# 0xWOLAND/halo2-prover

Hardware: AMD Instinct MI355X
Metric: MSM+NTT field-ops/s (higher is better)
Workload: dtype u32 limbs (256-bit modular)

## Files before the change

halo2_prover_amd/csrc/h2_msm.hpp:

```cpp
#pragma once
#include "h2_curve29.hpp"
#include "h2_curve_quad.hpp"
#include "h2_tune.hpp"
#include <hip/hip_ext.h>
#include <algorithm>
#include <cstdlib>

namespace h2 {

#ifdef H2_TAIL_STAMPS
__device__ unsigned long long* h2_stamps;
#define H2_STAMP(slot)                                                                                              \
  do {                                                                                                              \
    if (threadIdx.x == 0) h2_stamps[((size_t)blockIdx.y * gridDim.x + blockIdx.x) * 16 + (slot)] = wall_clock64(); \
  } while (0)
#else
#define H2_STAMP(slot)
#endif

constexpr uint32_t MSM_SIGN = 0x80000000u;
constexpr uint32_t MSM_MAX_WINDOWS = 48;
constexpr uint32_t MSM_HOT_SPAN = 256;
constexpr uint32_t MSM_HOT_SEG = 128;
constexpr uint32_t MSM_NOT_HOT = 0xFFFFFFFFu;
constexpr uint32_t MSM_SORT_THREADS = 1024;
constexpr uint32_t MSM_CHUNK_WAVES = 3;
constexpr uint32_t MSM_MAX_C_ONE_LEVEL = 16;
constexpr uint32_t MSM_MAX_C = 19;

struct MsmGeom {
  uint32_t c;
  uint32_t W;
  uint32_t B;
  uint32_t nbits;
  uint32_t wbase, wextra;
  uint8_t off[MSM_MAX_WINDOWS];
  uint8_t width[MSM_MAX_WINDOWS];
};

inline MsmGeom msm_geometry(size_t n, uint32_t nbits) {
  uint32_t lg = 0;
  while (((size_t)1 << (lg + 1)) <= n) lg++;
  int c = (int)lg - (lg <= 15 ? 3 : 4);
  c = lg <= 20 ? std::min(c, 16) : 19;
  c = tune_int("H2_TUNE_C", c);
  if (c < 6) c = 6;
  if (c > (int)MSM_MAX_C) c = (int)MSM_MAX_C;
  MsmGeom g{};
  g.nbits = nbits;
  const uint32_t total = nbits + 1;
  g.W = (total + c - 1) / c;
  const uint32_t base = total / g.W, extra = total % g.W;
  g.wbase = base;
  g.wextra = extra;
  uint32_t o = 0;
  for (uint32_t w = 0; w < g.W; w++) {
    g.off[w] = (uint8_t)o;
    g.width[w] = (uint8_t)(base + (w < extra ? 1 : 0));
    o += g.width[w];
  }
  g.c = base + (extra ? 1 : 0);
  g.B = 1u << (g.c - 1);
  return g;
}

constexpr size_t MSM_TABLE_SCRATCH = 80;
template <class CV>
__global__ void __launch_bounds__(256)
msm_table_kernel(const U128* __restrict__ bases, U128* __restrict__ table, uint32_t* __restrict__ scratch, uint32_t n, MsmGeom g,
                 uint32_t* __restrict__ bad) {
  const uint32_t i = blockIdx.x * blockDim.x + threadIdx.x;
  if (i >= n) return;
  using B = typename CV::Base;
  using W = Fe29<B>;
  Affine<CV> p = affine_load<CV>(bases + 4 * (size_t)i);
  if (!p.is_identity()) {
    Fe<B> b;
#pragma unroll
    for (int k = 0; k < 8; k++) b.v[k] = CV::B(k);
    uint32_t rx[8], ry[8];
    fe_reduce_once<B>(rx, p.x.v, 0);
    fe_reduce_once<B>(ry, p.y.v, 0);
    bool ok = true;
#pragma unroll
    for (int k = 0; k < 8; k++) ok = ok && rx[k] == p.x.v[k] && ry[k] == p.y.v[k];
    if (!ok || fe_sqr(p.y) != fe_add(fe_mul(fe_sqr(p.x), p.x), b)) {
      atomicAdd(bad, 1u);
      p = Affine<CV>::identity();
    }
  }
  if (p.is_identity()) {
    for (uint32_t w = 0; w < g.W; w++) affine29_store_table<CV>(table + 4 * ((size_t)w * n + i), p);
    return;
  }
  auto slot_of = [&](uint32_t w) { return reinterpret_cast<uint32_t*>(table + 4 * ((size_t)w * n + i)); };
  auto scr_of = [&](uint32_t w) { return scratch + (MSM_TABLE_SCRATCH / 4) * ((size_t)w * n + i); };
  auto put9 = [](uint32_t* q, const W& v) {
#pragma unroll
    for (int l = 0; l < 9; l++) q[l] = (uint32_t)v.v[l];
  };
  auto get9 = [](const uint32_t* q) {
    W v;
#pragma unroll
    for (int l = 0; l < 9; l++) v.v[l] = (int32_t)q[l];
    return v;
  };
// ... 433 lines not shown
  return affine29_load<CV>(table + 4 * (size_t)(entry & ~MSM_SIGN), (entry & MSM_SIGN) != 0);
}

template <class CV>
__global__ void __launch_bounds__(256, MSM_CHUNK_WAVES)
msm_chunk_kernel(const U128* __restrict__ table, const U128* const* __restrict__ col_tables, uint32_t log_b,
                 const uint32_t* __restrict__ sorted_ref,
                 const uint32_t* __restrict__ chunk_first, const uint32_t* __restrict__ offsets, size_t K, uint32_t T_host,
                 uint32_t* __restrict__ bucket_sum, uint32_t* __restrict__ head, uint32_t* __restrict__ tail) {
  const uint32_t t = blockIdx.x * blockDim.x + threadIdx.x;
  const uint32_t E = offsets[K];
  const uint32_t T = msm_effective_t(E, T_host);
  const uint64_t lo64 = (uint64_t)t * T;
  if (lo64 >= E) return;
  const uint32_t lo = (uint32_t)lo64, hi = (uint32_t)min((uint64_t)E, lo64 + T);
  uint32_t key = chunk_first[t];
  uint32_t next = offsets[key + 1];
  if (col_tables) table = col_tables[key >> log_b];
  bool first = true;
  Xyzz29<CV> a = Xyzz29<CV>::identity();
  U128 quad = U128{0, 0, 0, 0};
  for (uint32_t e = lo; e < hi; e++) {
    if (e == lo || (e & 3u) == 0) quad = *reinterpret_cast<const U128*>(sorted_ref + (e & ~3u));
    const uint32_t sel = e & 3u;
    const uint32_t ref = sel == 0 ? quad.x : sel == 1 ? quad.y : sel == 2 ? quad.z : quad.w;
    if (e >= next) {
      if (first && offsets[key] != lo) xyzz29_store<CV>(head + XYZZ29_WORDS * (size_t)t, a);
      else xyzz29_store<CV>(bucket_sum + XYZZ29_WORDS * (size_t)key, a);
      first = false;
      a = Xyzz29<CV>::identity();
      do {
        key++;
        next = offsets[key + 1];
      } while (e >= next);
      if (col_tables) table = col_tables[key >> log_b];
    }
    a = xyzz29_add_affine(a, msm_fetch<CV>(table, ref));
  }
  const bool ends_here = next == hi;
  const bool starts_here = !first || offsets[key] == lo;
  if (starts_here && ends_here) xyzz29_store<CV>(bucket_sum + XYZZ29_WORDS * (size_t)key, a);
  else if (first) xyzz29_store<CV>(head + XYZZ29_WORDS * (size_t)t, a);
  else xyzz29_store<CV>(tail + XYZZ29_WORDS * (size_t)t, a);
}

template <class CV>
__device__ __forceinline__ Xyzz29<CV> xyzz_shfl_down(const Xyzz29<CV>& p, uint32_t delta) {
  Xyzz29<CV> r;
#pragma unroll
  for (int i = 0; i < 9; i++) {
    r.x.v[i] = __shfl_down(p.x.v[i], delta, 64);
    r.y.v[i] = __shfl_down(p.y.v[i], delta, 64);
    r.zz.v[i] = __shfl_down(p.zz.v[i], delta, 64);
    r.zzz.v[i] = __shfl_down(p.zzz.v[i], delta, 64);
  }
  return r;
}

__device__ __forceinline__ void h2_publish_release() {
  asm volatile("s_waitcnt vmcnt(0)" ::: "memory");
  __builtin_amdgcn_fence(__ATOMIC_RELEASE, "agent");
  asm volatile("s_waitcnt vmcnt(0)" ::: "memory");
}
__device__ __forceinline__ void h2_consume_acquire() {
  __builtin_amdgcn_fence(__ATOMIC_ACQUIRE, "agent");
  asm volatile("s_waitcnt vmcnt(0)" ::: "memory");
}

template <class CV>
__device__ __forceinline__ Xyzz29<CV> xyzz_fold_down(const Xyzz29<CV>& a, uint32_t d, uint32_t lane) {
  const Xyzz29<CV> o = xyzz_shfl_down(a, d);
  return lane < d ? xyzz29_add_quad(a, o) : a;
}

template <class CV>
__device__ __forceinline__ Xyzz29<CV> msm_piece(const uint32_t* __restrict__ head, const uint32_t* __restrict__ tail,
                                               uint32_t s, uint32_t j0, uint32_t T, uint32_t p) {
  const uint32_t j = j0 + p;
  const uint32_t* src = (p == 0 && s != j0 * T) ? tail : head;
  return xyzz29_load<CV>(src + XYZZ29_WORDS * (size_t)j);
}

template <class CV>
__global__ void __launch_bounds__(64)
msm_hot_reduce_kernel(const uint32_t* __restrict__ offsets, size_t K, uint32_t T_host, const uint32_t* __restrict__ hot_slot,
                      const uint32_t* __restrict__ tasks, const uint32_t* __restrict__ task_count, uint32_t max_tasks,
                      const uint32_t* __restrict__ head, const uint32_t* __restrict__ tail, uint32_t* __restrict__ hot_part) {
  __builtin_amdgcn_s_setprio(3);
  const uint32_t ntask = min(*task_count, max_tasks);
  const uint32_t T = msm_effective_t(offsets[K], T_host);
  const uint32_t quad = threadIdx.x >> 2;
  for (uint32_t t = blockIdx.x; t < ntask; t += gridDim.x) {
    const uint32_t key = tasks[2 * t], q = tasks[2 * t + 1];
    const uint32_t s = offsets[key], e = offsets[key + 1];
    const uint32_t j0 = s / T, span = (e - 1) / T - j0 + 1;
    const uint32_t lo = q * MSM_HOT_SEG, hi = min(span, lo + MSM_HOT_SEG);
    Xyzz29<CV> a = Xyzz29<CV>::identity();
    for (uint32_t p = lo + quad; p < hi; p += 16) a = xyzz29_add_quad(a, msm_piece<CV>(head, tail, s, j0, T, p));
    for (uint32_t d = 32; d >= 4; d >>= 1) a = xyzz_fold_down(a, d, threadIdx.x);
    if (threadIdx.x == 0) xyzz29_store<CV>(hot_part + XYZZ29_WORDS * (size_t)(hot_slot[key] + q), a);
  }
}

template <class CV>
__global__ void __launch_bounds__(256)
msm_fixup_kernel(const uint32_t* __restrict__ offsets, size_t K, uint32_t T_host, uint32_t log_g,
                 const uint32_t* __restrict__ bucket_sum, const uint32_t* __restrict__ head,
                 const uint32_t* __restrict__ tail, const uint32_t* __restrict__ hot_slot,
                 const uint32_t* __restrict__ hot_part, uint32_t* __restrict__ xsum) {
  __builtin_amdgcn_s_setprio(3);
  const uint32_t G = 1u << log_g;
  const uint32_t T = msm_effective_t(offsets[K], T_host);
  const size_t gt = (size_t)blockIdx.x * blockDim.x + threadIdx.x;
  const size_t key = gt >> log_g;
  const uint32_t lane = (uint32_t)gt & (G - 1);
  const uint32_t quad = lane >> 2, nquad = G >> 2;
  const bool live = key < K;
  Xyzz29<CV> x = Xyzz29<CV>::identity();
  if (live) {
    const uint32_t s = offsets[key], e = offsets[key + 1];
    if (e > s) {
      const uint32_t j0 = s / T, j1 = (e - 1) / T;
      if (j0 == j1) {
        if (quad == 0) x = xyzz29_load<CV>(bucket_sum + XYZZ29_WORDS * key);
      } else if (hot_slot[key] != MSM_NOT_HOT) {
        const uint32_t nseg = (j1 - j0 + 1 + MSM_HOT_SEG - 1) / MSM_HOT_SEG;
        const uint32_t* part = hot_part + XYZZ29_WORDS * (size_t)hot_slot[key];
        for (uint32_t q = quad; q < nseg; q += nquad) x = xyzz29_add_quad(x, xyzz29_load<CV>(part + XYZZ29_WORDS * (size_t)q));
      } else if (quad <= j1 - j0) {
        Xyzz29<CV> nxt = msm_piece<CV>(head, tail, s, j0, T, quad);
        for (uint32_t p = quad; p <= j1 - j0; p += nquad) {
          const Xyzz29<CV> cur = nxt;
          if (p + nquad <= j1 - j0) nxt = msm_piece<CV>(head, tail, s, j0, T, p + nquad);
          x = xyzz29_add_quad(x, cur);
        }
      }
    }
  }
  for (uint32_t d = G >> 1; d >= 4; d >>= 1) x = xyzz_fold_down(x, d, lane);
  if (live && lane == 0) xyzz29_store<CV>(xsum + XYZZ29_WORDS * key, x);
}

H2_HD bool msm_special_predoubled(uint32_t log_b, uint32_t lb) {
  const uint32_t hb = log_b - lb, ndig = ((hb + 1) >> 1) ? ((hb + 1) >> 1) : 1u;
  return lb >= 2 * ndig;
}
template <class CV>
__global__ void __launch_bounds__(256)
msm_rowcol_kernel(const uint32_t* __restrict__ xsum, uint32_t* __restrict__ rc, uint32_t* __restrict__ done,
                  uint32_t log_b, uint32_t lb, U128* zero_ptr = nullptr, uint32_t zero_u128 = 0) {
  __builtin_amdgcn_s_setprio(3);
  __shared__ uint32_t xw[3][XYZZ29_WORDS];
  const uint32_t col = blockIdx.y;
  if (blockIdx.x == 0 && threadIdx.x == 0) done[col] = 0;
  if (zero_ptr) {
    const uint32_t nthr = gridDim.x * gridDim.y * blockDim.x;
    for (uint32_t i = (blockIdx.y * gridDim.x + blockIdx.x) * blockDim.x + threadIdx.x; i < zero_u128; i += nthr)
      zero_ptr[i] = U128{0, 0, 0, 0};
  }
  const uint32_t rows = 1u << (log_b - lb), cols = 1u << lb;
  const bool is_row = blockIdx.x < rows;
  const uint32_t first = is_row ? blockIdx.x * cols : blockIdx.x - rows;
  const uint32_t stride = is_row ? 1u : cols, len = is_row ? cols : rows;
  const uint32_t* base = xsum + XYZZ29_WORDS * ((size_t)col << log_b);
  const uint32_t quad = threadIdx.x >> 2, nq = blockDim.x >> 2, lane = threadIdx.x & 63u, wave = threadIdx.x >> 6;
  Xyzz29<CV> a = quad < len ? xyzz29_load<CV>(base + XYZZ29_WORDS * (size_t)(first + quad * stride)) : Xyzz29<CV>::identity();
  if (quad + nq < len) {
    Xyzz29<CV> nxt = xyzz29_load<CV>(base + XYZZ29_WORDS * (size_t)(first + (quad + nq) * stride));
    for (uint32_t j = quad + nq; j < len; j += nq) {
      const Xyzz29<CV> cur = nxt;
      if (j + nq < len) nxt = xyzz29_load<CV>(base + XYZZ29_WORDS * (size_t)(first + (j + nq) * stride));
      a = xyzz29_add_quad(a, cur);
    }
  }
  for (uint32_t d = 32; d >= 4; d >>= 1) a = xyzz_fold_down(a, d, lane);
  if (blockDim.x > 64) {
    if (wave > 0 && lane == 0) xyzz29_store<CV>(xw[wave - 1], a);
    __syncthreads();
    if (wave > 0) return;
    const uint32_t nw = blockDim.x >> 6;
    if (quad >= 1) a = quad < nw ? xyzz29_load<CV>(xw[quad - 1]) : Xyzz29<CV>::identity();
    for (uint32_t d = 2 * nw; d >= 4; d >>= 1) a = xyzz_fold_down(a, d, lane);
  }
  if (is_row || (blockIdx.x == rows + cols - 1 && msm_special_predoubled(log_b, lb)))
    for (uint32_t k = 0; k < lb; k++) a = xyzz29_double_quad(a);
  if (threadIdx.x == 0) xyzz29_store<CV>(rc + XYZZ29_WORDS * ((size_t)col * (rows + cols) + blockIdx.x), a);
}
inline uint32_t msm_rowcol_waves(uint32_t log_b, uint32_t lb, size_t m) {
  const uint32_t rows = 1u << (log_b - lb), cols = 1u << lb;
  const uint32_t shortest = rows < cols ? rows : cols;
  uint32_t nw = 1;
  while (nw < 4 && shortest >= 64 * nw && (size_t)(rows + cols) * m * (2 * nw) <= 1024) nw *= 2;
  return nw;
}

template <class CV>
__device__ __forceinline__ Xyzz29<CV> xyzz29_pick(uint32_t dig, const Xyzz29<CV>& p1, const Xyzz29<CV>& p2, const Xyzz29<CV>& p3) {
  const int32_t m1 = -(int32_t)(dig == 1), m2 = -(int32_t)(dig == 2), m3 = -(int32_t)(dig == 3);
  Xyzz29<CV> r;
#pragma unroll
  for (int i = 0; i < 9; i++) {
    r.x.v[i] = (m1 & p1.x.v[i]) | (m2 & p2.x.v[i]) | (m3 & p3.x.v[i]);
    r.y.v[i] = (m1 & p1.y.v[i]) | (m2 & p2.y.v[i]) | (m3 & p3.y.v[i]);
    r.zz.v[i] = (m1 & p1.zz.v[i]) | (m2 & p2.zz.v[i]) | (m3 & p3.zz.v[i]);
    r.zzz.v[i] = (m1 & p1.zzz.v[i]) | (m2 & p2.zzz.v[i]) | (m3 & p3.zzz.v[i]);
  }
  return r;
}

constexpr uint32_t MSM_FINAL_MAX_BLOCKS = 64;
H2_HD uint32_t msm_final_row_blocks(uint32_t log_b, uint32_t lb) { return ((1u << (log_b - lb)) + 15u) / 16u; }
H2_HD uint32_t msm_final_blocks(uint32_t log_b, uint32_t lb) {
  return msm_final_row_blocks(log_b, lb) + ((1u << lb) - 1u + 15u) / 16u;
}
template <class CV>
__global__ void __launch_bounds__(64)
msm_final_kernel(const uint32_t* __restrict__ rc, uint32_t* part , uint32_t* done,
// ... 164 lines not shown
  uint32_t arrived = 0;
  if (threadIdx.x == 0) {
    xyzz29_store<CV>(part + XYZZ29_WORDS * (size_t)blockIdx.x, r);
    h2_publish_release();
    arrived = atomicAdd(counter + job, 1u);
  }
  arrived = __shfl(arrived, 0, 64);
  if (arrived != gridDim.x - 1) return;
  h2_consume_acquire();
  Xyzz29<CV> acc = Xyzz29<CV>::identity();
  for (uint32_t b = quad; b < gridDim.x; b += 16) acc = xyzz29_add_quad(acc, xyzz29_load<CV>(part + XYZZ29_WORDS * (size_t)b));
  for (uint32_t d = 32; d >= 4; d >>= 1) acc = xyzz_fold_down(acc, d, threadIdx.x);
  if (threadIdx.x == 0) {
    Fe<B> jx, jy, jz;
    xyzz_to_jacobian(xyzz29_to_api(acc), jx, jy, jz);
    fe_store<B>(out_jac + 6 * (size_t)job, jx);
    fe_store<B>(out_jac + 6 * (size_t)job + 2, jy);
    fe_store<B>(out_jac + 6 * (size_t)job + 4, jz);
  }
}

template <class CV>
__global__ void __launch_bounds__(256)
srs_powers_kernel(U128* __restrict__ out, Fe<typename CV::Scalar> s, uint32_t n) {
  const uint32_t i = blockIdx.x * blockDim.x + threadIdx.x;
  if (i >= n) return;
  using FS = typename CV::Scalar;
  using FB = typename CV::Base;
  Fe<FS> k = fe_from_mont(fe_pow_u64(s, (uint64_t)i));
  Affine<CV> g;
#pragma unroll
  for (int j = 0; j < 8; j++) {
    g.x.v[j] = CV::GX(j);
    g.y.v[j] = CV::GY(j);
  }
  Xyzz<CV> r = Xyzz<CV>::identity();
  for (int bit = 255; bit >= 0; bit--) {
    r = xyzz_double(r);
    if ((k.v[bit >> 5] >> (bit & 31)) & 1) r = xyzz_add_affine(r, g);
  }
  Affine<CV> a = xyzz_to_affine(r);
  fe_store<FB>(out + 4 * (size_t)i, a.x);
  fe_store<FB>(out + 4 * (size_t)i + 2, a.y);
}

template <class CV>
__global__ void __launch_bounds__(256)
fixed_base_mul_kernel(U128* __restrict__ out, const U128* __restrict__ scalars, uint32_t n) {
  const uint32_t i = blockIdx.x * blockDim.x + threadIdx.x;
  if (i >= n) return;
  using FS = typename CV::Scalar;
  using FB = typename CV::Base;
  Fe<FS> k = fe_from_mont(fe_load<FS>(scalars + 2 * (size_t)i));
  Affine<CV> g;
#pragma unroll
  for (int j = 0; j < 8; j++) {
    g.x.v[j] = CV::GX(j);
    g.y.v[j] = CV::GY(j);
  }
  Xyzz<CV> r = Xyzz<CV>::identity();
  for (int bit = 255; bit >= 0; bit--) {
    r = xyzz_double(r);
    if ((k.v[bit >> 5] >> (bit & 31)) & 1) r = xyzz_add_affine(r, g);
  }
  Affine<CV> a = xyzz_to_affine(r);
  fe_store<FB>(out + 4 * (size_t)i, a.x);
  fe_store<FB>(out + 4 * (size_t)i + 2, a.y);
}

constexpr uint32_t MSM_WS_REGIONS = 32;
constexpr uint8_t MSM_GUARD_BYTE = 0xA5;
struct MsmRegion {
  const char* name;
  size_t off, bytes;
};
struct MsmWorkspace {
  size_t n, m;
  size_t K;
  size_t E;
  size_t nblk;
  uint32_t T;
  size_t nchunks;
  uint32_t log_g;
  uint32_t tile;
  uint32_t staged;
  size_t stage_lds;
  uint32_t sort2;
  Sort2Geom s2;
  uint32_t lb;
  uint32_t rc;
  size_t off_counts, off_gcounts, off_offsets, off_tile_base, off_tile_hist, off_blocksums, off_ref, off_key, off_misc, off_bsum,
      off_head, off_tail, off_xsum, off_rc, off_part, off_done, off_tree2, off_hot_slot, off_hot_tasks, off_hot_part, total;
  size_t off_cstart, off_group_base, off_mid_ref, off_mid_lo;
  size_t zero_bytes;
  uint32_t max_tasks;
  uint32_t guard;
  uint32_t n_regions;
  MsmRegion regions[MSM_WS_REGIONS];
};
inline size_t h2_align256(size_t x) { return (x + 255) & ~(size_t)255; }

inline bool msm_use_sort2(size_t n, size_t m, const MsmGeom& g) {
  const int forced = tune_int("H2_TUNE_SORT2", -1);
  const Sort2Geom s = msm_sort2_geom(n, g);
  const bool fits = g.B >= S2_MAX_F / 8 && s.F <= S2_MAX_F && (size_t)s.Hc * m <= S2_MAX_H;
  if (forced >= 0) return forced != 0 && fits;
  return fits && g.B > 4096;
}

inline MsmWorkspace msm_workspace(size_t n, size_t m, const MsmGeom& g, uint32_t guard = 0, size_t n_bases = 0,
                                  bool allow_pack = true) {
  if (!n_bases) n_bases = n;
  MsmWorkspace ws{};
  ws.n = n;
  ws.m = m;
  ws.guard = guard;
  ws.K = m * g.B;
  ws.E = m * g.W * n;
  ws.nblk = (ws.K + SCAN_BLOCK - 1) / SCAN_BLOCK;
  const uint64_t t_max = (uint64_t)tune_int("H2_TUNE_TMAX", 64);
  uint64_t T = t_max;
  {
    uint64_t best = ~0ull;
    for (uint64_t w = MSM_CHUNK_WAVES; w >= 2; w--) {
      uint64_t t = (ws.E + w * 65536 - 1) / (w * 65536);
      if (t < 8) t = 8;
      if (t > t_max) continue;
      const uint64_t cost = w * t * (w == 2 ? 21 : 20);
      if (cost < best) { best = cost; T = t; }
    }
  }
  ws.T = (uint32_t)T;
  ws.nchunks = (ws.E + T - 1) / T;
  {
    const size_t fine = std::min<size_t>((ws.E + 7) / 8, (size_t)MSM_CHUNK_WAVES * 65536 + 1);
    if (ws.nchunks < fine) ws.nchunks = fine;
  }
  const double span = (double)g.W * (double)n / (double)g.B / (double)T + 1.0;
  uint32_t lq = 0;
  while ((1u << lq) < span && lq < 4) lq++;
  while (lq > 0 && (ws.K << lq) > 40960) lq--;
  lq = (uint32_t)tune_int("H2_TUNE_LQ", (int)lq);
  uint32_t lg = lq + 2;
  ws.log_g = lg;
  ws.sort2 = msm_use_sort2(n, m, g) ? 1u : 0u;
  ws.s2 = msm_sort2_geom(n, g, allow_pack ? n_bases : 0);
  size_t tile = (n * m + 1023) / 1024;
  const size_t dense = (size_t)2 * g.B / g.W;
  if (tile < dense) tile = dense;
  if (tile < 256) tile = 256;
  tile *= (size_t)tune_int("H2_TUNE_TILE_MUL", 2);
  if (tile > n) tile = n;
  ws.staged = 0;
  ws.stage_lds = 0;
  if (!ws.sort2) {
    const size_t cap = 160 * 1024 - 512;
    auto need = [&](size_t t) { return (size_t)8 * g.B + (size_t)6 * t * g.W + 64; };
    if (g.B <= 65536 && n * m >= 8192 && need(dense) <= cap) {
      for (size_t rounds = 1; rounds <= 2; rounds++) {
        size_t t = (n * m + 256 * rounds - 1) / (256 * rounds);
        if (t < dense) t = dense;
        if (t < 256) t = 256;
        if (t > n) t = n;
        if (need(t) <= cap) {
          tile = t;
          ws.staged = 1;
          ws.stage_lds = need(t);
          break;
        }
      }
    }
  }
  ws.tile = (uint32_t)tile;
  ws.lb = (g.c - 1) / 2;
  ws.rc = (1u << (g.c - 1 - ws.lb)) + (1u << ws.lb);
  size_t o = 0;
  auto region = [&](const char* name, size_t bytes) {
    const size_t at = o;
    if (ws.n_regions < MSM_WS_REGIONS) ws.regions[ws.n_regions++] = MsmRegion{name, at, bytes};
    o = h2_align256(o + bytes) + (guard ? h2_align256(guard) : 0);
    return at;
  };
  const size_t tiles = (n + ws.tile - 1) / ws.tile;
  if (ws.sort2) {
    const size_t H = (size_t)ws.s2.Hc * m, t2 = (size_t)ws.s2.tiles * m;
    ws.zero_bytes = 256 + H * 4;
    ws.off_misc = region("zeroed: misc + coarse counters", ws.zero_bytes);
    ws.off_gcounts = ws.off_misc + 256;
    ws.off_counts = ws.off_gcounts;
    ws.off_cstart = region("coarse bin starts", (H + 1) * 4);
    ws.off_offsets = region("offsets", (ws.K + 1) * 4);
    ws.off_tile_base = region("tile bases", t2 * ws.s2.Hc * 4);
    ws.off_tile_hist = region("tile counts", t2 * ws.s2.Hc * 4);
    ws.off_group_base = region("group bases", (size_t)ws.s2.groups * m * ws.s2.Hc * 4);
    ws.off_mid_ref = region("coarse-sorted entries", ws.E * 4);
    ws.off_mid_lo = region("coarse-sorted low key bits", ws.s2.pack_shift ? 0 : ws.E);
    ws.off_blocksums = ws.off_cstart;
  } else {
    ws.zero_bytes = 256 + h2_align256(ws.K * 4) + MSM_XCDS * ws.K * 4;
    ws.off_misc = region("zeroed: misc + counts + group counters", ws.zero_bytes);
    ws.off_counts = ws.off_misc + 256;
    ws.off_gcounts = ws.off_counts + h2_align256(ws.K * 4);
    ws.off_offsets = region("offsets", (ws.K + 1) * 4);
    ws.off_tile_base = region("tile bases", tiles * ws.K * 4);
    ws.off_tile_hist = region("tile counts", ws.staged ? tiles * ws.K * 4 : 0);
    ws.off_blocksums = region("scan block sums", (ws.nblk + 1) * 4);
  }
  ws.off_ref = region("sorted entries", ws.E * 4 + 16);
  ws.off_key = region("chunk first keys", (ws.nchunks + 1) * 4);
  ws.off_bsum = region("bucket sums", ws.K * (XYZZ29_WORDS * 4));
  ws.off_head = region("chunk heads", ws.nchunks * (XYZZ29_WORDS * 4));
  ws.off_tail = region("chunk tails", ws.nchunks * (XYZZ29_WORDS * 4));
  ws.off_xsum = region("bucket point sums", ws.K * (XYZZ29_WORDS * 4));
  ws.off_rc = region("row / column sums", m * ws.rc * (XYZZ29_WORDS * 4));
  ws.off_part = region("final partials", m * MSM_FINAL_MAX_BLOCKS * (XYZZ29_WORDS * 4));
  ws.off_done = region("final counters", m * 4);
  ws.off_tree2 = region("results", m * (XYZZ29_WORDS * 4));
  ws.max_tasks = (uint32_t)(ws.nchunks / MSM_HOT_SEG + 2 * (ws.nchunks / MSM_HOT_SPAN) + 16);
  ws.off_hot_slot = region("hot slots", ws.K * 4);
  ws.off_hot_tasks = region("hot tasks", (size_t)ws.max_tasks * 8);
  ws.off_hot_part = region("hot partials", (size_t)ws.max_tasks * (XYZZ29_WORDS * 4));
  ws.total = o;
  return ws;
}

#define MSM_REQUIRE(cond) \
  do {                    \
    if (!(cond)) return #cond; \
  } while (0)
inline const char* msm_check(const MsmWorkspace& ws, const MsmGeom& g, size_t n, size_t m, size_t col_stride,
                             uint32_t n_bases, size_t arena_bytes) {
  auto bytes_at = [&](size_t off) -> size_t {
    for (uint32_t r = 0; r < ws.n_regions; r++)
      if (off >= ws.regions[r].off && off < ws.regions[r].off + ws.regions[r].bytes)
        return ws.regions[r].off + ws.regions[r].bytes - off;
    return 0;
  };
  MSM_REQUIRE(ws.n == n && ws.m == m);
  MSM_REQUIRE(n >= 1 && m >= 1 && n <= n_bases);
  MSM_REQUIRE(m == 1 || col_stride >= n);
  MSM_REQUIRE(ws.n_regions < MSM_WS_REGIONS);
  MSM_REQUIRE(ws.total <= arena_bytes);
  for (uint32_t r = 0; r + 1 < ws.n_regions; r++)
    MSM_REQUIRE(ws.regions[r].off + ws.regions[r].bytes + ws.guard <= ws.regions[r + 1].off);
  MSM_REQUIRE(ws.regions[ws.n_regions - 1].off + ws.regions[ws.n_regions - 1].bytes + ws.guard <= ws.total);
  MSM_REQUIRE(g.W >= 1 && g.W <= MSM_MAX_WINDOWS && g.B == (1u << (g.c - 1)) && g.c <= MSM_MAX_C);
  MSM_REQUIRE(ws.sort2 || g.c <= MSM_MAX_C_ONE_LEVEL);
  MSM_REQUIRE((uint64_t)g.W * n_bases < (1ull << 31));
  MSM_REQUIRE(ws.K == m * (size_t)g.B && ws.E == m * (size_t)g.W * n);
  MSM_REQUIRE(ws.E < (1ull << 31) && ws.K < (1ull << 31));
  MSM_REQUIRE(bytes_at(ws.off_misc) >= ws.zero_bytes && ws.zero_bytes >= 256);
  MSM_REQUIRE(ws.zero_bytes % 16 == 0 && ws.off_misc % 16 == 0 && ws.zero_bytes / 16 < (1ull << 32));
  MSM_REQUIRE(bytes_at(ws.off_offsets) >= (ws.K + 1) * 4);
  if (ws.sort2) {
    const Sort2Geom& s = ws.s2;
    const size_t H = (size_t)s.Hc * m;
    MSM_REQUIRE(s.F * s.Hc == g.B && s.F == (1u << s.lo_bits) && s.F <= S2_MAX_F && s.Hc <= S2_MAX_HC && H <= S2_MAX_H);
    MSM_REQUIRE(s.tile >= 1 && s.tile <= S2_THREADS && (size_t)s.tile * g.W <= S2_STAGE);
    MSM_REQUIRE((size_t)s.tiles * s.tile >= n && (size_t)(s.tiles - 1) * s.tile < n);
    MSM_REQUIRE(s.tiles <= 0x7FFFFFFFu && m <= 65535);
    MSM_REQUIRE(ws.off_gcounts == ws.off_misc + 256 && ws.zero_bytes >= 256 + H * 4);
    MSM_REQUIRE(bytes_at(ws.off_cstart) >= (H + 1) * 4);
    MSM_REQUIRE(bytes_at(ws.off_tile_base) >= (size_t)s.tiles * m * s.Hc * 4);
    MSM_REQUIRE(bytes_at(ws.off_tile_hist) >= (size_t)s.tiles * m * s.Hc * 4);
    MSM_REQUIRE(bytes_at(ws.off_mid_ref) >= ws.E * 4 && (s.pack_shift || bytes_at(ws.off_mid_lo) >= ws.E));
    MSM_REQUIRE(s.group >= 1 && s.group <= S2_GROUP && (size_t)s.groups * s.group >= s.tiles && bytes_at(ws.off_group_base) >= (size_t)s.groups * m * s.Hc * 4);
    MSM_REQUIRE(!s.pack_shift || (((uint64_t)g.W * n_bases <= (1ull << s.pack_shift)) && s.pack_shift + s.lo_bits <= 31));
    MSM_REQUIRE((size_t)s.Hc * 8 <= 64 * 1024);
    MSM_REQUIRE(msm_sort2_lds_scatter(s, g) <= 160 * 1024 - 512 && msm_sort2_lds_fine() + 4 * S2_MAX_F * 4 <= 160 * 1024 - 512);
  } else {
    const size_t tiles = (n + ws.tile - 1) / ws.tile;
    MSM_REQUIRE(ws.tile >= 1 && tiles * m < (1ull << 31) - MSM_XCDS);
    MSM_REQUIRE(msm_tile_grid((uint32_t)tiles, (uint32_t)m) >= tiles * m);
    MSM_REQUIRE((size_t)g.B * 4 <= 128 * 1024);
    MSM_REQUIRE(ws.off_counts == ws.off_misc + 256 && ws.off_gcounts >= ws.off_counts + ws.K * 4);
    MSM_REQUIRE(ws.off_gcounts + MSM_XCDS * ws.K * 4 <= ws.off_misc + ws.zero_bytes);
    MSM_REQUIRE(bytes_at(ws.off_tile_base) >= tiles * ws.K * 4);
    if (ws.staged) {
      MSM_REQUIRE(bytes_at(ws.off_tile_hist) >= tiles * ws.K * 4);
      MSM_REQUIRE(g.B <= 65536);
      MSM_REQUIRE(ws.stage_lds >= (size_t)8 * g.B + (size_t)6 * ws.tile * g.W && ws.stage_lds <= 160 * 1024 - 512);
    }
    if (ws.K > SCAN_LDS_MAX) {
      MSM_REQUIRE(ws.nblk * SCAN_BLOCK >= ws.K && ws.nblk < (1ull << 31));
      MSM_REQUIRE(bytes_at(ws.off_blocksums) >= (ws.nblk + 1) * 4);
    }
  }
  MSM_REQUIRE(bytes_at(ws.off_ref) >= ((ws.E + 3) & ~(size_t)3) * 4);
  MSM_REQUIRE(ws.T >= 8 && ws.nchunks >= (ws.E + ws.T - 1) / ws.T);
  MSM_REQUIRE(ws.nchunks >= std::min<size_t>((ws.E + 7) / 8, (size_t)MSM_CHUNK_WAVES * 65536 + 1));
  MSM_REQUIRE((ws.nchunks + 255) / 256 < (1ull << 31));
  MSM_REQUIRE(bytes_at(ws.off_key) >= ws.nchunks * 4);
  MSM_REQUIRE(bytes_at(ws.off_head) >= ws.nchunks * (XYZZ29_WORDS * 4) && bytes_at(ws.off_tail) >= ws.nchunks * (XYZZ29_WORDS * 4));
  MSM_REQUIRE(bytes_at(ws.off_bsum) >= ws.K * (XYZZ29_WORDS * 4) && bytes_at(ws.off_xsum) >= ws.K * (XYZZ29_WORDS * 4));
  MSM_REQUIRE(ws.log_g >= 2 && ws.log_g <= 6 && ((ws.K << ws.log_g) + 255) / 256 < (1ull << 31));
  MSM_REQUIRE(ws.lb < g.c && ws.rc == (1u << (g.c - 1 - ws.lb)) + (1u << ws.lb));
  MSM_REQUIRE(bytes_at(ws.off_rc) >= m * ws.rc * (XYZZ29_WORDS * 4));
  MSM_REQUIRE(msm_final_blocks(g.c - 1, ws.lb) <= MSM_FINAL_MAX_BLOCKS);
  MSM_REQUIRE(bytes_at(ws.off_part) >= m * MSM_FINAL_MAX_BLOCKS * (XYZZ29_WORDS * 4));
  MSM_REQUIRE(bytes_at(ws.off_done) >= m * 4 && bytes_at(ws.off_tree2) >= m * (XYZZ29_WORDS * 4));
  MSM_REQUIRE(bytes_at(ws.off_hot_slot) >= ws.K * 4);
  MSM_REQUIRE(bytes_at(ws.off_hot_tasks) >= (size_t)ws.max_tasks * 8);
  MSM_REQUIRE(bytes_at(ws.off_hot_part) >= (size_t)ws.max_tasks * (XYZZ29_WORDS * 4));
  MSM_REQUIRE(m <= 65535);
  return nullptr;
}
#undef MSM_REQUIRE

static __global__ void __launch_bounds__(256)
msm_guard_check_kernel(const uint8_t* __restrict__ arena, MsmWorkspace ws, uint32_t* __restrict__ bad ) {
  const uint32_t r = blockIdx.x;
  const size_t from = ws.regions[r].off + ws.regions[r].bytes;
  const size_t to = r + 1 < ws.n_regions ? ws.regions[r + 1].off : ws.total;
  uint32_t c = 0;
  for (size_t i = from + threadIdx.x; i < to; i += blockDim.x) c += arena[i] != MSM_GUARD_BYTE;
  if (c) atomicAdd(&bad[r], c);
}

template <class CV>
inline hipError_t msm_kernel_setup() {
  hipError_t e;
  const int lds = (int)((1u << (MSM_MAX_C_ONE_LEVEL - 1)) * 4);
  if ((e = hipFuncSetAttribute((const void*)msm_digits_kernel<CV>, hipFuncAttributeMaxDynamicSharedMemorySize, lds)) != hipSuccess) return e;
  if ((e = hipFuncSetAttribute((const void*)msm_scatter_kernel<CV>, hipFuncAttributeMaxDynamicSharedMemorySize, lds)) != hipSuccess) return e;
  if ((e = hipFuncSetAttribute((const void*)msm_scatter_staged_kernel<CV>, hipFuncAttributeMaxDynamicSharedMemorySize, 160 * 1024 - 512)) != hipSuccess) return e;
  if ((e = hipFuncSetAttribute((const void*)msm2_scatter_kernel<CV>, hipFuncAttributeMaxDynamicSharedMemorySize, 160 * 1024 - 512)) != hipSuccess) return e;
  if ((e = hipFuncSetAttribute((const void*)msm2_fine_kernel, hipFuncAttributeMaxDynamicSharedMemorySize, (int)msm_sort2_lds_fine())) != hipSuccess) return e;
  return hipFuncSetAttribute((const void*)scan_lds_kernel, hipFuncAttributeMaxDynamicSharedMemorySize, (int)(SCAN_LDS_MAX * 4));
}

template <class CV>
inline hipError_t msm_launch(const U128* table, const U128* const* per_column ,
                             uint32_t n_bases, const U128* d_scalars, size_t n, size_t col_stride,
                             size_t m, const MsmGeom& g, char* ws_base, const MsmWorkspace& ws, hipStream_t stream,
                             hipEvent_t ev_start = nullptr, hipEvent_t ev_stop = nullptr, hipEvent_t ev_tail = nullptr,
                             U128* d_out_jac = nullptr ,
                             bool zeroed = false ) {
  uint32_t* counts = (uint32_t*)(ws_base + ws.off_counts);
  uint32_t* gcounts = (uint32_t*)(ws_base + ws.off_gcounts);
  uint32_t* offsets = (uint32_t*)(ws_base + ws.off_offsets);
  uint32_t* tile_base = (uint32_t*)(ws_base + ws.off_tile_base);
  uint32_t* blocksums = (uint32_t*)(ws_base + ws.off_blocksums);
  uint32_t* sref = (uint32_t*)(ws_base + ws.off_ref);
  uint32_t* chunk_first = (uint32_t*)(ws_base + ws.off_key);
  uint32_t* misc = (uint32_t*)(ws_base + ws.off_misc);
  uint32_t* bsum = (uint32_t*)(ws_base + ws.off_bsum);
  uint32_t* head = (uint32_t*)(ws_base + ws.off_head);
  uint32_t* tail = (uint32_t*)(ws_base + ws.off_tail);
  uint32_t* xsum = (uint32_t*)(ws_base + ws.off_xsum);
  uint32_t* rc = (uint32_t*)(ws_base + ws.off_rc);
  uint32_t* tree2 = (uint32_t*)(ws_base + ws.off_tree2);
  uint32_t* hot_slot = (uint32_t*)(ws_base + ws.off_hot_slot);
  uint32_t* hot_tasks = (uint32_t*)(ws_base + ws.off_hot_tasks);
  uint32_t* hot_part = (uint32_t*)(ws_base + ws.off_hot_part);
  hipError_t e;
  if (per_column && m > MSM_MAX_MULTI) return hipErrorInvalidValue;
  if (!zeroed && (e = hipMemsetAsync(misc, 0, ws.zero_bytes, stream)) != hipSuccess) return e;
  uint32_t* tile_hist = (ws.staged || ws.sort2) ? (uint32_t*)(ws_base + ws.off_tile_hist) : nullptr;
  const U128** d_tables = nullptr;
  uint32_t log_b = 0;
  MsmKeysArgs keys_args{};
  keys_args.chunk_first = chunk_first;
  keys_args.hot_slot = hot_slot;
  keys_args.tasks = hot_tasks;
  keys_args.task_count = misc;
  keys_args.max_tasks = ws.max_tasks;
  keys_args.T_host = ws.T;
  if (per_column) {
    d_tables = (const U128**)(misc + 16);
    keys_args.n_tables = (uint32_t)m;
    keys_args.tables_dst = d_tables;
    for (size_t j = 0; j < m; j++) keys_args.tables.t[j] = per_column[j];
    while ((1u << log_b) < g.B) log_b++;
  }
  bool keys_merged = false;
  if (ws.sort2) {
    const Sort2Geom& s2 = ws.s2;
    const uint32_t H = s2.Hc * (uint32_t)m;
    uint32_t* cstart = (uint32_t*)(ws_base + ws.off_cstart);
    uint32_t* mid_ref = (uint32_t*)(ws_base + ws.off_mid_ref);
    uint8_t* mid_lo = (uint8_t*)(ws_base + ws.off_mid_lo);
    uint32_t* group_base = (uint32_t*)(ws_base + ws.off_group_base);
    hipLaunchKernelGGL(msm2_count_kernel<CV>, dim3(s2.groups, (unsigned)m), dim3(S2_THREADS), (size_t)s2.Hc * 8, stream, d_scalars,
                       gcounts, tile_base, tile_hist, group_base, (uint32_t)n, col_stride, s2, g);
    hipLaunchKernelGGL(msm2_coarse_scan_kernel, dim3(1), dim3(1024), 0, stream, gcounts, cstart, H, offsets + ws.K);
    hipLaunchKernelGGL(msm2_scatter_kernel<CV>, dim3(s2.tiles, (unsigned)m), dim3(S2_THREADS), msm_sort2_lds_scatter(s2, g), stream,
                       d_scalars, cstart, tile_base, tile_hist, group_base, mid_ref, mid_lo, (uint32_t)n, col_stride, n_bases, s2, g);
    hipLaunchKernelGGL(msm2_fine_kernel, dim3(H), dim3(S2_THREADS), msm_sort2_lds_fine(), stream, cstart, mid_ref, mid_lo, sref,
                       offsets, s2.F, s2.lo_bits, s2.pack_shift);
  } else {
    const size_t lds = (size_t)g.B * 4;
    const uint32_t tiles = (uint32_t)((n + ws.tile - 1) / ws.tile);
    const uint32_t sort_grid = msm_tile_grid(tiles, (uint32_t)m);
    hipLaunchKernelGGL(msm_digits_kernel<CV>, dim3(sort_grid), dim3(MSM_SORT_THREADS), lds, stream, d_scalars, gcounts,
                       tile_base, tile_hist, (uint32_t)n, col_stride, ws.tile, tiles, (uint32_t)m, g);
    if (ws.K <= SCAN_LDS_MAX) {
      uint32_t per = (uint32_t)((ws.K + 1023) / 1024);
      per |= 1u;
      hipLaunchKernelGGL(scan_lds_kernel, dim3(1), dim3(1024), ws.K * 4, stream, gcounts, offsets, (uint32_t)ws.K, per);
    } else {
      hipLaunchKernelGGL(msm_group_fold_kernel, dim3((unsigned)((ws.K + 255) / 256)), dim3(256), 0, stream, gcounts, counts, ws.K);
      hipLaunchKernelGGL(scan_reduce_kernel, dim3((unsigned)ws.nblk), dim3(256), 0, stream, counts, blocksums, ws.K);
      hipLaunchKernelGGL(scan_blocksums_kernel, dim3(1), dim3(1024), 0, stream, blocksums, (uint32_t)ws.nblk, misc + 1);
      hipLaunchKernelGGL(scan_apply_kernel, dim3((unsigned)ws.nblk), dim3(256), 0, stream, counts, blocksums, offsets,
                         ws.K);
    }
    if (ws.staged) {
      const size_t per = (ws.K + (size_t)tiles * m - 1) / ((size_t)tiles * m);
      keys_merged = per <= MSM_SORT_THREADS && ws.stage_lds >= (size_t)4 * (MSM_SORT_THREADS + 1);
      MsmKeysArgs ka = keys_args;
      const uint32_t grid = sort_grid;
      if (keys_merged) ka.keys_per_block = (uint32_t)per;
      hipLaunchKernelGGL(msm_scatter_staged_kernel<CV>, dim3(grid), dim3(MSM_SORT_THREADS), ws.stage_lds, stream, d_scalars,
                         offsets, gcounts, tile_base, tile_hist, sref, (uint32_t)n, col_stride, n_bases, ws.tile, tiles,
                         (uint32_t)m, g, (uint32_t)(ws.tile * g.W), ka);
    } else
      hipLaunchKernelGGL(msm_scatter_kernel<CV>, dim3(sort_grid), dim3(MSM_SORT_THREADS), lds, stream, d_scalars, offsets,
                         gcounts, tile_base, sref, (uint32_t)n, col_stride, n_bases, ws.tile, tiles, (uint32_t)m, g);
  }
  if (!keys_merged)
    hipLaunchKernelGGL(msm_keys_kernel, dim3((unsigned)((ws.K + MSM_KEYS_THREADS - 1) / MSM_KEYS_THREADS)), dim3(MSM_KEYS_THREADS), 0,
                       stream, (const uint32_t*)offsets, ws.K, keys_args);
  hipEvent_t ev_end = ev_stop ? ev_stop : ev_tail;
  if (ev_start || ev_end)
    hipExtLaunchKernelGGL(msm_chunk_kernel<CV>, dim3((unsigned)((ws.nchunks + 255) / 256)), dim3(256), 0, stream, ev_start, ev_end,
                          0, table, (const U128* const*)d_tables, log_b, (const uint32_t*)sref, (const uint32_t*)chunk_first,
                          (const uint32_t*)offsets, ws.K, ws.T, bsum, head, tail);
  else
    hipLaunchKernelGGL(msm_chunk_kernel<CV>, dim3((unsigned)((ws.nchunks + 255) / 256)), dim3(256), 0, stream, table,
                       (const U128* const*)d_tables, log_b, sref, chunk_first, offsets, ws.K, ws.T, bsum, head, tail);
  if (ev_stop && ev_tail) (void)hipEventRecord(ev_tail, stream);
  hipLaunchKernelGGL(msm_hot_reduce_kernel<CV>, dim3(1024), dim3(64), 0, stream, offsets, ws.K, ws.T, hot_slot, hot_tasks,
                     misc, ws.max_tasks, head, tail, hot_part);
  const size_t fix_threads = ws.K << ws.log_g;
  hipLaunchKernelGGL(msm_fixup_kernel<CV>, dim3((unsigned)((fix_threads + 255) / 256)), dim3(256), 0, stream, offsets,
                     ws.K, ws.T, ws.log_g, bsum, head, tail, hot_slot, hot_part, xsum);
  uint32_t* part = (uint32_t*)(ws_base + ws.off_part);
  uint32_t* done = (uint32_t*)(ws_base + ws.off_done);
  hipLaunchKernelGGL(msm_rowcol_kernel<CV>, dim3(ws.rc, (unsigned)m), dim3(64 * msm_rowcol_waves(g.c - 1, ws.lb, m)), 0, stream,
                     xsum, rc, done, g.c - 1, ws.lb, (U128*)misc, (uint32_t)(ws.zero_bytes / 16));
  hipLaunchKernelGGL(msm_final_kernel<CV>, dim3(msm_final_blocks(g.c - 1, ws.lb), (unsigned)m), dim3(64), 0, stream, rc, part,
                     done, tree2, d_out_jac, g.c - 1, ws.lb);
  return hipGetLastError();
}

}
```

Baseline: 179.2 billion.

## Add per-thread bucket piece partials kernel merged with hot reduce before fixup

Replaces the hot-reduce kernel with a combined partials kernel. Extra blocks handle the hot tasks, four waves per block. The remaining threads each sum a strided subset of a bucket's chunk pieces into a new piece-partials buffer using single-thread point adds. The fixup kernel then folds at most S values per bucket (partials or raw pieces) instead of walking every piece, and the group size lq is now derived from S. The aim is to spread the long per-bucket piece chains over more threads. The cost is an extra workspace region, extra global writes and reads, and a heuristic for S.

```diff
diff --git a/halo2_prover_amd/csrc/h2_msm.hpp b/halo2_prover_amd/csrc/h2_msm.hpp
--- a/halo2_prover_amd/csrc/h2_msm.hpp
+++ b/halo2_prover_amd/csrc/h2_msm.hpp
@@ -22,6 +22,8 @@
 constexpr uint32_t MSM_MAX_WINDOWS = 48;
 constexpr uint32_t MSM_HOT_SPAN = 256;
 constexpr uint32_t MSM_HOT_SEG = 128;
+constexpr uint32_t MSM_HOT_BLOCKS = 256;
+constexpr uint32_t MSM_MAX_PS = 16;
 constexpr uint32_t MSM_NOT_HOT = 0xFFFFFFFFu;
 constexpr uint32_t MSM_SORT_THREADS = 1024;
 constexpr uint32_t MSM_CHUNK_WAVES = 3;
@@ -621,32 +623,53 @@
 }
 
 template <class CV>
-__global__ void __launch_bounds__(64)
-msm_hot_reduce_kernel(const uint32_t* __restrict__ offsets, size_t K, uint32_t T_host, const uint32_t* __restrict__ hot_slot,
-                      const uint32_t* __restrict__ tasks, const uint32_t* __restrict__ task_count, uint32_t max_tasks,
-                      const uint32_t* __restrict__ head, const uint32_t* __restrict__ tail, uint32_t* __restrict__ hot_part) {
+__global__ void __launch_bounds__(256)
+msm_partials_kernel(const uint32_t* __restrict__ offsets, uint32_t K, uint32_t T_host, uint32_t S,
+                    const uint32_t* __restrict__ hot_slot, const uint32_t* __restrict__ tasks,
+                    const uint32_t* __restrict__ task_count, uint32_t max_tasks, const uint32_t* __restrict__ head,
+                    const uint32_t* __restrict__ tail, uint32_t* __restrict__ hot_part, uint32_t* __restrict__ part) {
   __builtin_amdgcn_s_setprio(3);
-  const uint32_t ntask = min(*task_count, max_tasks);
   const uint32_t T = msm_effective_t(offsets[K], T_host);
-  const uint32_t quad = threadIdx.x >> 2;
-  for (uint32_t t = blockIdx.x; t < ntask; t += gridDim.x) {
-    const uint32_t key = tasks[2 * t], q = tasks[2 * t + 1];
-    const uint32_t s = offsets[key], e = offsets[key + 1];
-    const uint32_t j0 = s / T, span = (e - 1) / T - j0 + 1;
-    const uint32_t lo = q * MSM_HOT_SEG, hi = min(span, lo + MSM_HOT_SEG);
-    Xyzz29<CV> a = Xyzz29<CV>::identity();
-    for (uint32_t p = lo + quad; p < hi; p += 16) a = xyzz29_add_quad(a, msm_piece<CV>(head, tail, s, j0, T, p));
-    for (uint32_t d = 32; d >= 4; d >>= 1) a = xyzz_fold_down(a, d, threadIdx.x);
-    if (threadIdx.x == 0) xyzz29_store<CV>(hot_part + XYZZ29_WORDS * (size_t)(hot_slot[key] + q), a);
-  }
+  const uint32_t lane_blocks = gridDim.x - MSM_HOT_BLOCKS;
+  if (blockIdx.x >= lane_blocks) {
+    const uint32_t ntask = min(*task_count, max_tasks);
+    const uint32_t lane = threadIdx.x & 63u, quad = lane >> 2;
+    for (uint32_t t = (blockIdx.x - lane_blocks) * 4 + (threadIdx.x >> 6); t < ntask; t += MSM_HOT_BLOCKS * 4) {
+      const uint32_t key = tasks[2 * t], q = tasks[2 * t + 1];
+      const uint32_t s = offsets[key], e = offsets[key + 1];
+      const uint32_t j0 = s / T, span = (e - 1) / T - j0 + 1;
+      const uint32_t lo = q * MSM_HOT_SEG, hi = min(span, lo + MSM_HOT_SEG);
+      Xyzz29<CV> a = Xyzz29<CV>::identity();
+      for (uint32_t p = lo + quad; p < hi; p += 16) a = xyzz29_add_quad(a, msm_piece<CV>(head, tail, s, j0, T, p));
+      for (uint32_t d = 32; d >= 4; d >>= 1) a = xyzz_fold_down(a, d, lane);
+      if (lane == 0) xyzz29_store<CV>(hot_part + XYZZ29_WORDS * (size_t)(hot_slot[key] + q), a);
+    }
+    return;
+  }
+  const uint32_t gt = blockIdx.x * blockDim.x + threadIdx.x;
+  const uint32_t key = gt / S, slot = gt - key * S;
+  if (key >= K) return;
+  const uint32_t s = offsets[key], e = offsets[key + 1];
+  if (e <= s) return;
+  const uint32_t j0 = s / T, np = (e - 1) / T - j0 + 1;
+  if (slot + S >= np) return;
+  if (np > MSM_HOT_SPAN && hot_slot[key] != MSM_NOT_HOT) return;
+  Xyzz29<CV> a = msm_piece<CV>(head, tail, s, j0, T, slot);
+  Xyzz29<CV> nxt = msm_piece<CV>(head, tail, s, j0, T, slot + S);
+  for (uint32_t p = slot + S; p < np; p += S) {
+    const Xyzz29<CV> cur = nxt;
+    if (p + S < np) nxt = msm_piece<CV>(head, tail, s, j0, T, p + S);
+    a = xyzz29_add(a, cur);
+  }
+  xyzz29_store<CV>(part + XYZZ29_WORDS * (size_t)gt, a);
 }
 
 template <class CV>
 __global__ void __launch_bounds__(256)
-msm_fixup_kernel(const uint32_t* __restrict__ offsets, size_t K, uint32_t T_host, uint32_t log_g,
+msm_fixup_kernel(const uint32_t* __restrict__ offsets, size_t K, uint32_t T_host, uint32_t log_g, uint32_t S,
                  const uint32_t* __restrict__ bucket_sum, const uint32_t* __restrict__ head,
                  const uint32_t* __restrict__ tail, const uint32_t* __restrict__ hot_slot,
-                 const uint32_t* __restrict__ hot_part, uint32_t* __restrict__ xsum) {
+                 const uint32_t* __restrict__ hot_part, const uint32_t* __restrict__ piece_part, uint32_t* __restrict__ xsum) {
   __builtin_amdgcn_s_setprio(3);
   const uint32_t G = 1u << log_g;
   const uint32_t T = msm_effective_t(offsets[K], T_host);
@@ -659,19 +682,26 @@
   if (live) {
     const uint32_t s = offsets[key], e = offsets[key + 1];
     if (e > s) {
-      const uint32_t j0 = s / T, j1 = (e - 1) / T;
-      if (j0 == j1) {
+      const uint32_t j0 = s / T, np = (e - 1) / T - j0 + 1;
+      if (np == 1) {
         if (quad == 0) x = xyzz29_load<CV>(bucket_sum + XYZZ29_WORDS * key);
-      } else if (hot_slot[key] != MSM_NOT_HOT) {
-        const uint32_t nseg = (j1 - j0 + 1 + MSM_HOT_SEG - 1) / MSM_HOT_SEG;
-        const uint32_t* part = hot_part + XYZZ29_WORDS * (size_t)hot_slot[key];
-        for (uint32_t q = quad; q < nseg; q += nquad) x = xyzz29_add_quad(x, xyzz29_load<CV>(part + XYZZ29_WORDS * (size_t)q));
-      } else if (quad <= j1 - j0) {
-        Xyzz29<CV> nxt = msm_piece<CV>(head, tail, s, j0, T, quad);
-        for (uint32_t p = quad; p <= j1 - j0; p += nquad) {
-          const Xyzz29<CV> cur = nxt;
-          if (p + nquad <= j1 - j0) nxt = msm_piece<CV>(head, tail, s, j0, T, p + nquad);
-          x = xyzz29_add_quad(x, cur);
+      } else {
+        const bool hot = np > MSM_HOT_SPAN && hot_slot[key] != MSM_NOT_HOT;
+        const uint32_t nval = hot ? (np + MSM_HOT_SEG - 1) / MSM_HOT_SEG : min(np, S);
+        const uint32_t* part = hot ? hot_part + XYZZ29_WORDS * (size_t)hot_slot[key] : piece_part + XYZZ29_WORDS * (key * S);
+        auto value = [&](uint32_t q) {
+          return (hot || q + S < np) ? xyzz29_load<CV>(part + XYZZ29_WORDS * (size_t)q) : msm_piece<CV>(head, tail, s, j0, T, q);
+        };
+        if (quad < nval) {
+          x = value(quad);
+          if (quad + nquad < nval) {
+            Xyzz29<CV> nxt = value(quad + nquad);
+            for (uint32_t q = quad + nquad; q < nval; q += nquad) {
+              const Xyzz29<CV> cur = nxt;
+              if (q + nquad < nval) nxt = value(q + nquad);
+              x = xyzz29_add_quad(x, cur);
+            }
+          }
         }
       }
     }
@@ -1002,6 +1032,7 @@
   uint32_t T;
   size_t nchunks;
   uint32_t log_g;
+  uint32_t ps;
   uint32_t tile;
   uint32_t staged;
   size_t stage_lds;
@@ -1010,7 +1041,7 @@
   uint32_t lb;
   uint32_t rc;
   size_t off_counts, off_gcounts, off_offsets, off_tile_base, off_tile_hist, off_blocksums, off_ref, off_key, off_misc, off_bsum,
-      off_head, off_tail, off_xsum, off_rc, off_part, off_done, off_tree2, off_hot_slot, off_hot_tasks, off_hot_part, total;
+      off_head, off_tail, off_xsum, off_rc, off_part, off_done, off_tree2, off_hot_slot, off_hot_tasks, off_hot_part, off_piece_part, total;
   size_t off_cstart, off_group_base, off_mid_ref, off_mid_lo;
   size_t zero_bytes;
   uint32_t max_tasks;
@@ -1057,8 +1088,13 @@
     if (ws.nchunks < fine) ws.nchunks = fine;
   }
   const double span = (double)g.W * (double)n / (double)g.B / (double)T + 1.0;
+  uint32_t ps = (uint32_t)std::min<size_t>(MSM_MAX_PS, 65536 / std::max<size_t>(ws.K, 1));
+  if ((double)ps > span / 2) ps = (uint32_t)(span / 2);
+  if (ps < 1) ps = 1;
+  ps = (uint32_t)std::clamp(tune_int("H2_TUNE_PS", (int)ps), 1, (int)MSM_MAX_PS);
+  ws.ps = ps;
   uint32_t lq = 0;
-  while ((1u << lq) < span && lq < 4) lq++;
+  while (((ps + (1u << lq) - 1) >> lq) > 5 && lq < 4) lq++;
   while (lq > 0 && (ws.K << lq) > 40960) lq--;
   lq = (uint32_t)tune_int("H2_TUNE_LQ", (int)lq);
   uint32_t lg = lq + 2;
@@ -1140,6 +1176,7 @@
   ws.off_hot_slot = region("hot slots", ws.K * 4);
   ws.off_hot_tasks = region("hot tasks", (size_t)ws.max_tasks * 8);
   ws.off_hot_part = region("hot partials", (size_t)ws.max_tasks * (XYZZ29_WORDS * 4));
+  ws.off_piece_part = region("piece partials", ws.K * ws.ps * (XYZZ29_WORDS * 4));
   ws.total = o;
   return ws;
 }
@@ -1222,6 +1259,9 @@
   MSM_REQUIRE(bytes_at(ws.off_hot_slot) >= ws.K * 4);
   MSM_REQUIRE(bytes_at(ws.off_hot_tasks) >= (size_t)ws.max_tasks * 8);
   MSM_REQUIRE(bytes_at(ws.off_hot_part) >= (size_t)ws.max_tasks * (XYZZ29_WORDS * 4));
+  MSM_REQUIRE(ws.ps >= 1 && ws.ps <= MSM_MAX_PS && (uint64_t)ws.K * ws.ps < (1ull << 32) - 256);
+  MSM_REQUIRE(bytes_at(ws.off_piece_part) >= ws.K * ws.ps * (XYZZ29_WORDS * 4));
+  MSM_REQUIRE((ws.K * ws.ps + 255) / 256 + MSM_HOT_BLOCKS < (1ull << 31));
   MSM_REQUIRE(m <= 65535);
   return nullptr;
 }
@@ -1273,6 +1313,7 @@
   uint32_t* hot_slot = (uint32_t*)(ws_base + ws.off_hot_slot);
   uint32_t* hot_tasks = (uint32_t*)(ws_base + ws.off_hot_tasks);
   uint32_t* hot_part = (uint32_t*)(ws_base + ws.off_hot_part);
+  uint32_t* piece_part = (uint32_t*)(ws_base + ws.off_piece_part);
   hipError_t e;
   if (per_column && m > MSM_MAX_MULTI) return hipErrorInvalidValue;
   if (!zeroed && (e = hipMemsetAsync(misc, 0, ws.zero_bytes, stream)) != hipSuccess) return e;
@@ -1350,11 +1391,11 @@
     hipLaunchKernelGGL(msm_chunk_kernel<CV>, dim3((unsigned)((ws.nchunks + 255) / 256)), dim3(256), 0, stream, table,
                        (const U128* const*)d_tables, log_b, sref, chunk_first, offsets, ws.K, ws.T, bsum, head, tail);
   if (ev_stop && ev_tail) (void)hipEventRecord(ev_tail, stream);
-  hipLaunchKernelGGL(msm_hot_reduce_kernel<CV>, dim3(1024), dim3(64), 0, stream, offsets, ws.K, ws.T, hot_slot, hot_tasks,
-                     misc, ws.max_tasks, head, tail, hot_part);
+  hipLaunchKernelGGL(msm_partials_kernel<CV>, dim3((unsigned)((ws.K * ws.ps + 255) / 256) + MSM_HOT_BLOCKS), dim3(256), 0, stream,
+                     offsets, (uint32_t)ws.K, ws.T, ws.ps, hot_slot, hot_tasks, misc, ws.max_tasks, head, tail, hot_part, piece_part);
   const size_t fix_threads = ws.K << ws.log_g;
   hipLaunchKernelGGL(msm_fixup_kernel<CV>, dim3((unsigned)((fix_threads + 255) / 256)), dim3(256), 0, stream, offsets,
-                     ws.K, ws.T, ws.log_g, bsum, head, tail, hot_slot, hot_part, xsum);
+                     ws.K, ws.T, ws.log_g, ws.ps, bsum, head, tail, hot_slot, hot_part, piece_part, xsum);
   uint32_t* part = (uint32_t*)(ws_base + ws.off_part);
   uint32_t* done = (uint32_t*)(ws_base + ws.off_done);
   hipLaunchKernelGGL(msm_rowcol_kernel<CV>, dim3(ws.rc, (unsigned)m), dim3(64 * msm_rowcol_waves(g.c - 1, ws.lb, m)), 0, stream,
```

New measurement: 181.4 billion, median of 6. +1.3%, better.
